# JessicaLeu-code/MotionPlanning_5D_m

Measured on AMD Instinct MI355X. Metric: CFS iterations/sec, 5-DoF 30-wp 8-obs batch-1024; l_inf wp err vs quadprog, higher is better.
Workload: dtype f64

## Files before the change

include/cfs_hip.h:

```cpp
#ifndef CFS_HIP_H
#define CFS_HIP_H

#ifdef __cplusplus
extern "C" {
#endif

#define CFS_ABI_VERSION 1
#define CFS_MAX_LINKS 8
#define CFS_MAX_OBS 32
#define CFS_MAX_H 64

typedef enum cfs_error {
    CFS_SUCCESS = 0,
    CFS_ERR_INVALID_ARG = -1,
    CFS_ERR_NO_DEVICE = -2,
    CFS_ERR_HIP = -3,
    CFS_ERR_NOT_SPD = -4,
    CFS_ERR_DYNAMICS = -5,
    CFS_ERR_ALLOC = -6
} cfs_error;

typedef enum cfs_status {
    CFS_OK_CONVERGED = 0,
    CFS_OK_MAXITER = 1,
// ... 295 lines not shown
int cfs_cart_path_mesh(const cfs_cart_desc *d, int nmesh, const cfs_mesh *const *meshes, const double *D_mesh, int flags, int T,
                       const double *start, const int *start_state, const double *target_pos, const double *target_axis,
                       const double *theta_ref, const cfs_cart_out *out);
int cfs_cart_path_mesh_device(const cfs_cart_desc *d, int nmesh, const cfs_mesh *const *meshes, const double *D_mesh ,
                              int flags, int T, const double *start, const int *start_state, const double *target_pos,
                              const double *target_axis, const double *theta_ref, const cfs_cart_out *out, void *stream);

int cfs_cart_follow(const cfs_cart_desc *d, int T, int npts, const double *start, const int *start_state, const double *path_pos,
                    const double *path_axis, const double *theta_ref, const cfs_cart_out *out);
int cfs_cart_follow_device(const cfs_cart_desc *d, int T, int npts, const double *start, const int *start_state, const double *path_pos,
                           const double *path_axis, const double *theta_ref, const cfs_cart_out *out, void *stream);
int cfs_cart_follow_mesh(const cfs_cart_desc *d, int nmesh, const cfs_mesh *const *meshes, const double *D_mesh, int flags, int T, int npts,
                         const double *start, const int *start_state, const double *path_pos, const double *path_axis,
                         const double *theta_ref, const cfs_cart_out *out);
int cfs_cart_follow_mesh_device(const cfs_cart_desc *d, int nmesh, const cfs_mesh *const *meshes, const double *D_mesh ,
                                int flags, int T, int npts, const double *start, const int *start_state, const double *path_pos,
                                const double *path_axis, const double *theta_ref, const cfs_cart_out *out, void *stream);

#define CFS_DBG_NO_REFINE 2
#define CFS_DBG_NO_WARM_START 8
#define CFS_DBG_NO_CERTIFICATE 16
#define CFS_DBG_NO_PRUNE 32
#define CFS_DBG_NO_AUTO_ORDER 64
#define CFS_DBG_TIER_W1 128
#define CFS_DBG_CLEAR_NO_BOUND 256
#define CFS_DBG_CLEAR_SEED 512
int cfs_debug_set_options(cfs_problem *p, int mask, int warm_max, double polish_tol);
int cfs_debug_fused_tier(int njoint, int H, int nobs, int mode, int per_waypoint, int limits, int force_w1, int *tier);
int cfs_debug_stamps(cfs_problem *p, int B, unsigned long long *out);
int cfs_debug_trace_begin(cfs_problem *p, int b, int cap);
int cfs_debug_trace_read(cfs_problem *p, double *out);
int cfs_debug_log_u(cfs_problem *p, int on);
int cfs_debug_read_u_log(cfs_problem *p, int B, double *out);
int cfs_debug_rrt_frontier_overflows(unsigned long long *count, int reset);
int cfs_debug_ik_frontier_overflows(unsigned long long *count, int reset);
int cfs_debug_cart_frontier_overflows(unsigned long long *count, int reset);

#ifdef __cplusplus
}
#endif
#endif
```

motionplanning_5d_m_amd/_lib.py:

```python
from __future__ import annotations

import ctypes as C
import os

try:
    import torch
except Exception:
    torch = None

_HERE = os.path.dirname(os.path.abspath(__file__))
LIB_PATH = os.path.join(_HERE, "libcfs_hip.so")

CFS_MAX_LINKS = 8
CFS_MAX_OBS = 32
CFS_MAX_H = 64

CFS_SUCCESS = 0
ERRORS = {-1: "CFS_ERR_INVALID_ARG", -2: "CFS_ERR_NO_DEVICE", -3: "CFS_ERR_HIP", -4: "CFS_ERR_NOT_SPD",
          -5: "CFS_ERR_DYNAMICS", -6: "CFS_ERR_ALLOC"}
STATUS = {0: "OK_CONVERGED", 1: "OK_MAXITER", 2: "QP_INFEASIBLE", 3: "NUMERIC", 4: "SOFT_ENDED"}
ROBOT_KIND = {"M16iB": 0, "M200i": 1, "2L": 2}
MODE = {"CFS": 0, "PSGCFS": 1}
JACOBIAN = {"fd_literal": 0, "analytic": 1}
INFEASIBLE = {"stop": 0, "soften": 1}
# ... 211 lines not shown
    ("cfs_solve_batch_device", C.c_int, [_P, C.POINTER(cfs_batch_in), C.POINTER(cfs_batch_out), _P]),
    ("cfs_set_state_cost", C.c_int, [_P, _P]),
    ("cfs_build_terms_device", C.c_int, [_P, C.c_int, _P, _P, _P, _P, _P, _P, _P]),
    ("cfs_build_terms_from_routes_device", C.c_int, [_P, C.c_int, _P, C.c_int, _P, _P, _P, _P, _P]),
    ("cfs_profile_enable", C.c_int, [_P, C.c_int]),
    ("cfs_profile_read", C.c_int, [_P, C.POINTER(C.c_double), C.POINTER(C.c_double), C.POINTER(C.c_int)]),
    ("cfs_dist_arm", C.c_int, [C.POINTER(cfs_robot), C.c_int, C.c_int, _P, C.c_int, _P, _P, _P, _P]),
    ("cfs_linearize", C.c_int, [_P, C.c_int, _P, _P, _P, _P, _P]),
    ("cfs_get_con", C.c_int, [_P, C.c_int, _P, _P, _P, _P, _P, _P]),
    ("cfs_qp", C.c_int, [_P, C.c_int, _P, _P, _P, _P, _P, _P, _P, _P, _P]),
    ("cfs_mesh_create", C.c_int, [_P, C.c_int, _P, C.c_int, C.POINTER(_P)]),
    ("cfs_mesh_load_stl", C.c_int, [C.c_char_p, C.c_double, C.c_int, C.POINTER(_P)]),
    ("cfs_mesh_info", C.c_int, [_P, C.POINTER(C.c_int), C.POINTER(C.c_int), C.POINTER(C.c_int), C.POINTER(C.c_double)]),
    ("cfs_mesh_destroy", None, [_P]),
    ("cfs_mesh_segment_distance", C.c_int, [_P, C.c_int, _P, _P, _P, _P]),
    ("cfs_dist_arm_mesh", C.c_int, [C.POINTER(cfs_robot), C.c_int, C.c_int, _P, _P, _P, _P, _P]),
    ("cfs_problem_set_meshes", C.c_int, [_P, C.c_int, _P]),
    ("cfs_problem_set_mesh_motion", C.c_int, [_P, _P]),
    ("cfs_chomp_batch", C.c_int, [_P, C.POINTER(cfs_batch_in), _P, _P, _P, C.POINTER(cfs_batch_out)]),
    ("cfs_build_terms_from_ragged_routes_device", C.c_int, [_P, C.c_int, _P, C.c_int, _P, _P, _P, _P, _P, _P]),
    ("cfs_rrt_grow", C.c_int, [C.POINTER(cfs_rrt_desc), C.c_int, C.POINTER(cfs_rrt_out)]),
    ("cfs_rrt_grow_device", C.c_int, [C.POINTER(cfs_rrt_desc), C.c_int, C.POINTER(cfs_rrt_out), _P]),
    ("cfs_rrt_grow_mesh", C.c_int, [C.POINTER(cfs_rrt_desc), C.c_int, _P, _P, C.c_int, C.c_int, C.POINTER(cfs_rrt_out)]),
    ("cfs_rrt_grow_mesh_device", C.c_int, [C.POINTER(cfs_rrt_desc), C.c_int, _P, _P, C.c_int, C.c_int, C.POINTER(cfs_rrt_out), _P]),
    ("cfs_cost_b", C.c_int, [_P, C.c_int, _P, _P, _P, _P]),
    ("cfs_get_cost", C.c_int, [_P, C.c_int, _P, _P, _P, _P]),
    ("cfs_debug_set_options", C.c_int, [_P, C.c_int, C.c_int, C.c_double]),
    ("cfs_debug_fused_tier", C.c_int, [C.c_int] * 7 + [C.POINTER(C.c_int)]),
    ("cfs_debug_stamps", C.c_int, [_P, C.c_int, _P]),
    ("cfs_debug_trace_begin", C.c_int, [_P, C.c_int, C.c_int]),
    ("cfs_debug_trace_read", C.c_int, [_P, _P]),
    ("cfs_debug_log_u", C.c_int, [_P, C.c_int]),
    ("cfs_debug_read_u_log", C.c_int, [_P, C.c_int, _P]),
    ("cfs_debug_rrt_frontier_overflows", C.c_int, [C.POINTER(C.c_ulonglong), C.c_int]),
    ("cfs_problem_set_jacobian", C.c_int, [_P, C.c_int]),
    ("cfs_problem_get_jacobian", C.c_int, [_P, C.POINTER(C.c_int)]),
    ("cfs_problem_set_infeasible_policy", C.c_int, [_P, C.c_int, C.c_double]),
    ("cfs_problem_get_infeasible_policy", C.c_int, [_P, C.POINTER(C.c_int), C.POINTER(C.c_double)]),
    ("cfs_soft_results", C.c_int, [_P, C.c_int, _P, _P]),
    ("cfs_dist_arm_grad", C.c_int, [C.POINTER(cfs_robot), C.c_int, C.c_int, _P, C.c_int, _P, _P, _P, _P]),
    ("cfs_select_best_device", C.c_int, [_P, C.c_int, C.c_int, _P, C.POINTER(cfs_batch_out), _P, C.POINTER(cfs_batch_out), _P, _P, _P, _P]),
    ("cfs_problem_set_obstacle_motion", C.c_int, [_P, C.c_int]),
    ("cfs_problem_get_obstacle_motion", C.c_int, [_P, C.POINTER(C.c_int)]),
    ("cfs_problem_set_joint_limits", C.c_int, [_P, _P, _P]),
    ("cfs_problem_get_joint_limits", C.c_int, [_P, C.POINTER(C.c_int), _P, _P]),
    ("cfs_clearance_device", C.c_int, [_P, C.c_int, C.c_int, _P, _P, _P, _P, _P, _P, _P, _P, _P, _P]),
    ("cfs_clearance", C.c_int, [_P, C.c_int, C.c_int, _P, _P, _P, _P, _P, _P, _P, _P, _P]),
    ("cfs_clearance_mesh_device", C.c_int, [_P, C.c_int, C.c_int, _P, _P, _P, _P, _P, _P, _P, _P, _P, _P, _P]),
    ("cfs_clearance_mesh", C.c_int, [_P, C.c_int, C.c_int, _P, _P, _P, _P, _P, _P, _P, _P, _P, _P]),
    ("cfs_clearance_mesh_motion_device", C.c_int, [_P, C.c_int, C.c_int, _P, _P, _P, _P, _P, _P, _P, _P, _P, _P, _P]),
    ("cfs_clearance_mesh_motion", C.c_int, [_P, C.c_int, C.c_int, _P, _P, _P, _P, _P, _P, _P, _P, _P, _P]),
    ("cfs_ik_solve", C.c_int, [C.POINTER(cfs_ik_desc), C.c_int, _P, _P, _P, C.POINTER(cfs_ik_out)]),
    ("cfs_ik_solve_device", C.c_int, [C.POINTER(cfs_ik_desc), C.c_int, _P, _P, _P, C.POINTER(cfs_ik_out), _P]),
    ("cfs_tool_pose", C.c_int, [C.POINTER(cfs_robot), C.c_int, _P, _P, C.c_int, _P, _P, _P, _P]),
    ("cfs_ik_solve_mesh", C.c_int, [C.POINTER(cfs_ik_desc), C.c_int, _P, _P, C.c_int, C.c_int, _P, _P, _P, C.POINTER(cfs_ik_out)]),
    ("cfs_ik_solve_mesh_device", C.c_int, [C.POINTER(cfs_ik_desc), C.c_int, _P, _P, C.c_int, C.c_int, _P, _P, _P, C.POINTER(cfs_ik_out), _P]),
    ("cfs_debug_ik_frontier_overflows", C.c_int, [C.POINTER(C.c_ulonglong), C.c_int]),
    ("cfs_cart_path", C.c_int, [C.POINTER(cfs_cart_desc), C.c_int, _P, _P, _P, _P, _P, C.POINTER(cfs_cart_out)]),
    ("cfs_cart_path_device", C.c_int, [C.POINTER(cfs_cart_desc), C.c_int, _P, _P, _P, _P, _P, C.POINTER(cfs_cart_out), _P]),
    ("cfs_cart_path_mesh", C.c_int, [C.POINTER(cfs_cart_desc), C.c_int, _P, _P, C.c_int, C.c_int, _P, _P, _P, _P, _P, C.POINTER(cfs_cart_out)]),
    ("cfs_cart_path_mesh_device", C.c_int, [C.POINTER(cfs_cart_desc), C.c_int, _P, _P, C.c_int, C.c_int, _P, _P, _P, _P, _P, C.POINTER(cfs_cart_out),
                                            _P]),
    ("cfs_debug_cart_frontier_overflows", C.c_int, [C.POINTER(C.c_ulonglong), C.c_int]),
    ("cfs_cart_follow", C.c_int, [C.POINTER(cfs_cart_desc), C.c_int, C.c_int, _P, _P, _P, _P, _P, C.POINTER(cfs_cart_out)]),
    ("cfs_cart_follow_device", C.c_int, [C.POINTER(cfs_cart_desc), C.c_int, C.c_int, _P, _P, _P, _P, _P, C.POINTER(cfs_cart_out), _P]),
    ("cfs_cart_follow_mesh", C.c_int, [C.POINTER(cfs_cart_desc), C.c_int, _P, _P, C.c_int, C.c_int, C.c_int, _P, _P, _P, _P, _P,
# ... 38 lines not shown
```

motionplanning_5d_m_amd/csrc/cfs_api.hip:

```cpp
#include "cfs_problem.h"
#include <cmath>
#include <cstdarg>
#include <cstdio>
#include <cstring>
#include <cstdlib>
#include <new>
#include <vector>

namespace {

thread_local char g_err[512] = "";
int g_device = 0;

int have_device()
{
    int n = 0;
    if (hipGetDeviceCount(&n) != hipSuccess) return 0;
    return n;
}

}

int cfs_fail(int code, const char *fmt, ...)
{
// ... 137 lines not shown
    if (FamilyRefusal r = check_double_integrator(nj, H, dt, desc->Aaug, desc->Baug)) return cfs_fail(r.code, "%s", r.text);
    if (have_device() == 0) return cfs_fail(CFS_ERR_NO_DEVICE, "no HIP device visible");
    FamilyMatrices fm;
    if (FamilyRefusal r = family_matrices(nj, H, dt, desc->mode, desc->QQ, fm)) return cfs_fail(r.code, "%s", r.text);
    cfs_problem *p = new (std::nothrow) cfs_problem();
    if (!p) return cfs_fail(CFS_ERR_ALLOC, "out of host memory");
    p->d = *desc;
    p->QQ_host.assign(desc->QQ, desc->QQ + (size_t)nn * nn);
    p->d.QQ = p->d.Aaug = p->d.Baug = p->d.lim = p->d.MAX_input = p->d.margin = nullptr;
    p->device = g_device;
    if (hipDeviceGetAttribute(&p->n_cu, hipDeviceAttributeMultiprocessorCount, g_device) != hipSuccess || p->n_cu < 1) p->n_cu = 256;
    p->nn = nn; p->ns = ns; p->nx = nx; p->lmax_vel = fm.lmax_vel; p->lmax_H = fm.lmax_H;
    cfs_build_dev_robot(desc->robot, p->hrobot);
    cfs_clear_build_rho(p->hrobot, nj, p->rho);
    const size_t Bm = (size_t)desc->max_batch;
    p->pool_n = (int)std::min<size_t>(Bm, (size_t)2 * p->n_cu);
    const size_t Pn = (size_t)p->pool_n;
    hipError_t e = hipSetDevice(p->device);
    auto up = [&](auto &buf, const auto *src, size_t count) { if (e == hipSuccess) e = buf.upload(src, count); };
    auto room = [&](auto &buf, size_t count) { if (e == hipSuccess) e = buf.alloc(count); };
    up(p->rb, &p->hrobot, 1); up(p->QQ, desc->QQ, (size_t)nn * nn); up(p->Hinv, fm.Hinv.data(), (size_t)nn * nn);
    up(p->M1n, fm.M1n.data(), (size_t)nn * nn); up(p->M2n, fm.M2n.data(), (size_t)nn * nn); up(p->Hq, fm.Hq.data(), (size_t)nn * nn);
    room(p->Pt, Pn * pt_stride(nn));
    room(p->lim, 3 * (size_t)nj);
    if (e == hipSuccess) e = hipMemcpy(p->lim.p, desc->lim, nj * sizeof(double), hipMemcpyHostToDevice);
    if (desc->mode == CFS_MODE_CFS) up(p->maxin, desc->MAX_input, nn);
    else if (e == hipSuccess) e = p->maxin.zeros(nn);
    up(p->margin, desc->margin, desc->nobs);
    room(p->x0, Bm * nn); room(p->qu, Bm * nn); room(p->dist, Bm * desc->nobs * H); room(p->grad, Bm * desc->nobs * H * nj);
    room(p->Yg, Pn * nn * nn);
    if (e == hipSuccess) e = p->pool_flag.zeros(Pn * 16);
    if (desc->mode == CFS_MODE_CFS) { room(p->u_hist, Bm * (size_t)desc->MAX_O_ITER * nn); room(p->qu_hist, Bm * (size_t)desc->MAX_O_ITER * nn); }
    room(p->noise_row, Bm); room(p->linkid, Bm * desc->nobs * H); room(p->order, Bm); room(p->okey, Bm); room(p->order_user, Bm);
    if (e != hipSuccess) {
        delete p;
        return cfs_fail(CFS_ERR_HIP, "device setup failed: %s", hipGetErrorString(e));
    }
    *out = p;
    return CFS_SUCCESS;
}

void cfs_problem_destroy(cfs_problem *p)
{
    if (!p) return;
    (void)hipSetDevice(p->device);
    delete p;
}

int cfs_problem_family(const cfs_problem *p, double *QQ, double *alpha)
{
    if (!p) return cfs_fail(CFS_ERR_INVALID_ARG, "NULL handle");
    if (QQ) memcpy(QQ, p->QQ_host.data(), p->QQ_host.size() * sizeof(double));
    if (alpha) *alpha = p->d.alpha;
    return CFS_SUCCESS;
}

int cfs_problem_create_from_weights(const cfs_problem_desc *desc, const cfs_cost_weights *w, cfs_problem **out)
{
    if (!desc || !w || !out) return cfs_fail(CFS_ERR_INVALID_ARG, "NULL argument");
    *out = nullptr;
    if (!w->Qp || !w->Qv || !w->Rblk) return cfs_fail(CFS_ERR_INVALID_ARG, "Qp/Qv/Rblk must be given");
    const int nj = desc->njoint, H = desc->H;
    if (nj < 2 || nj > 6 || H < 1 || H > CFS_MAX_H) return cfs_fail(CFS_ERR_INVALID_ARG, "njoint %d / H %d unsupported", nj, H);
    const double dt = desc->robot.delta_t;
    if (!(dt > 0)) return cfs_fail(CFS_ERR_INVALID_ARG, "robot.delta_t must be positive");
    WeightFamily wf;
// ... 87 lines not shown
int cfs_solve_batch_device(cfs_problem *p, const cfs_batch_in *in, const cfs_batch_out *out, void *stream)
{
    if (!p || !in || !out) return cfs_fail(CFS_ERR_INVALID_ARG, "NULL argument");
    const int B = in->B;
    if (int rc = cfs_check_batch(p, B)) return rc;
    if (!in->x_init || !in->xR1 || !in->ff || !in->caug || !in->obs) return cfs_fail(CFS_ERR_INVALID_ARG, "NULL input array");
    if (!out->u || !out->x_ || !out->cost_all || !out->e_cost_all || !out->e_u_all || !out->iter_O || !out->total_iter || !out->status)
        return cfs_fail(CFS_ERR_INVALID_ARG, "NULL output array");
    CFS_HIPCHK(hipSetDevice(p->device));
    hipStream_t s = reinterpret_cast<hipStream_t>(stream);

    hipEvent_t e4[4] = {nullptr, nullptr, nullptr, nullptr};
    int rc = CFS_SUCCESS;
    if (p->prof)
        for (int k = 0; k < 4 && rc == CFS_SUCCESS; ++k) {
            if (!p->ev_free.empty()) { e4[k] = p->ev_free.back(); p->ev_free.pop_back(); }
            else if (hipEventCreate(&e4[k]) != hipSuccess) { e4[k] = nullptr; rc = cfs_fail(CFS_ERR_HIP, "hipEventCreate failed"); }
        }
    if (rc == CFS_SUCCESS) {
        rc = enqueue_solve(p, in, out, s, e4);
        if (rc != CFS_SUCCESS) p->pool_dirty = true;
    }
    if (p->prof)
        for (int k = 0; k < 4; ++k)
            if (e4[k]) (rc == CFS_SUCCESS ? p->ev : p->ev_free).push_back(e4[k]);
    return rc;
}

static int enqueue_solve(cfs_problem *p, const cfs_batch_in *in, const cfs_batch_out *out, hipStream_t s, hipEvent_t *e4)
{
    const int B = in->B, nj = p->d.njoint, nn = p->nn, K = p->d.MAX_O_ITER;
    if (p->pool_dirty) {
        CFS_HIPCHK(hipMemsetAsync(p->pool_flag.p, 0, (size_t)p->pool_n * 16 * sizeof(int), s));
        p->pool_dirty = false;
    }
    if (p->prof) CFS_HIPCHK(hipEventRecord(e4[0], s));
    if (p->d.mode == CFS_MODE_CFS) {
        GemvParams g;
        g.B = B; g.nn = nn; g.M = p->Hinv.p; g.X = in->ff; g.Y = p->x0.p; g.scale = -1.0;
        launch_batched_gemv(g, s);
    }
    if (p->prof) CFS_HIPCHK(hipEventRecord(e4[1], s));
    FusedParams fp;
    fill_fused_family(p, fp, B);
    fp.noise_rows = in->noise ? in->noise_rows : 0;
    fp.x_init = in->x_init; fp.xR1 = in->xR1; fp.ff = in->ff; fp.caug = in->caug; fp.obs = in->obs; fp.noise = in->noise;
    fp.u = out->u; fp.x_ = out->x_; fp.cost_all = out->cost_all; fp.e_cost_all = out->e_cost_all; fp.e_u_all = out->e_u_all;
    fp.iter_O = out->iter_O; fp.total_iter = out->total_iter; fp.status = out->status;
    fp.u_hist = (p->d.mode == CFS_MODE_CFS && K > 0) ? p->u_hist.p : nullptr;
    const int nline = p->d.nobs - p->nmesh;
    if (p->order_mode == 1 && p->order_n == B) fp.order = p->order_user.p;
    else if (p->order_mode != 2 && !(p->dbg_mask & CFS_DBG_NO_AUTO_ORDER) && B > p->n_cu && nline > 0) {
        OrderParams op;
        op.rb = p->rb.p; op.B = B; op.H = p->d.H; op.nj = nj; op.nobs = nline; op.obs_stride = p->d.nobs;
        op.wp_stride = cfs_moving(p) ? p->d.nobs : 0;
        op.x_init = in->x_init; op.obs = in->obs; op.margin = p->margin.p; op.key = p->okey.p; op.order = p->order.p;
        launch_order(op, s);
        fp.order = p->order.p;
    }
    SoftParams sp;
    const SoftParams *soft = soft_params(p, sp, true);
    if (p->soft_viol.p) {
        CFS_HIPCHK(hipMemsetAsync(p->soft_viol.p, 0, (size_t)B * std::max(K, 1) * sizeof(double), s));
        CFS_HIPCHK(hipMemsetAsync(p->soft_n.p, 0, (size_t)B * sizeof(int), s));
    }
    if (p->prof) CFS_HIPCHK(hipEventRecord(e4[2], s));
    if (p->nmesh == 0) {
        CFS_HIPCHK(launch_fused(nj, fp, s, force_w1(p), analytic(p), soft, cfs_moving(p), limited(p)));
    } else {
        LinMeshParams lm = lin_mesh_params(p, B);
        fp.nmesh = p->nmesh; fp.ext_dist = p->dist.p; fp.ext_grad = p->grad.p; fp.max_launch_iters = 1;
        fp.st_qu = p->qu.p; fp.st_cost = p->mesh.st_cost.p; fp.st_noise = p->noise_row.p; fp.st_done = p->mesh.st_done.p;
        for (int it = 0; it < std::max(K, 1); ++it) {
            lm.x_ = it == 0 ? in->x_init : out->x_;
            lm.status_done = it == 0 ? nullptr : p->mesh.st_done.p;
            lm.seed_prev = it > 0;
            CFS_HIPCHK(launch_linearize_mesh(nj, lm, s));
            fp.resume = it > 0;
            CFS_HIPCHK(launch_fused(nj, fp, s, force_w1(p), analytic(p), nullptr, false, limited(p)));
        }
    }
    if (p->prof) CFS_HIPCHK(hipEventRecord(e4[3], s));
    if (fp.u_hist) {
        if (p->u_hist.n) {
            GemvParams g;
            g.B = B * K; g.nn = nn; g.M = p->QQ.p; g.X = p->u_hist.p; g.Y = p->qu_hist.p; g.scale = 1.0;
            launch_batched_gemv(g, s);
            CostHistParams ch;
            ch.B = B; ch.nn = nn; ch.max_o_iter = K; ch.u_hist = p->u_hist.p; ch.qu_hist = p->qu_hist.p;
            ch.ff = in->ff; ch.caug = in->caug; ch.iter_O = out->iter_O; ch.cost_all = out->cost_all; ch.e_cost_all = out->e_cost_all;
// ... 154 lines not shown
    return CFS_SUCCESS;
}

int cfs_debug_trace_read(cfs_problem *p, double *out)
{
    if (!p || !out) return cfs_fail(CFS_ERR_INVALID_ARG, "NULL argument");
    if (!p->trace.p) return cfs_fail(CFS_ERR_INVALID_ARG, "no trace was begun");
    CFS_HIPCHK(hipSetDevice(p->device));
    CFS_HIPCHK(hipDeviceSynchronize());
    CFS_HIPCHK(hipMemcpy(out, p->trace.p, (size_t)(p->trace_cap + 1) * 8 * sizeof(double), hipMemcpyDeviceToHost));
    return CFS_SUCCESS;
}

int cfs_debug_log_u(cfs_problem *p, int on)
{
    if (!p) return cfs_fail(CFS_ERR_INVALID_ARG, "NULL handle");
    CFS_HIPCHK(hipSetDevice(p->device));
    CFS_HIPCHK(hipDeviceSynchronize());
    p->u_log.release();
    if (!on || p->d.MAX_O_ITER < 1) return CFS_SUCCESS;
    const size_t n = (size_t)p->d.max_batch * p->d.MAX_O_ITER * p->nn;
    CFS_HIPCHK(p->u_log.zeros(n));
    return CFS_SUCCESS;
}

int cfs_debug_read_u_log(cfs_problem *p, int B, double *out)
{
    if (!p || !out) return cfs_fail(CFS_ERR_INVALID_ARG, "NULL argument");
    if (!p->u_log.p) return cfs_fail(CFS_ERR_INVALID_ARG, "the u log is not enabled");
    if (int rc = cfs_check_batch(p, B)) return rc;
    CFS_HIPCHK(hipSetDevice(p->device));
    CFS_HIPCHK(hipDeviceSynchronize());
    CFS_HIPCHK(hipMemcpy(out, p->u_log.p, (size_t)B * p->d.MAX_O_ITER * p->nn * sizeof(double), hipMemcpyDeviceToHost));
    return CFS_SUCCESS;
}

int cfs_set_state_cost(cfs_problem *p, const double *Qaug)
{
    if (!p || !Qaug) return cfs_fail(CFS_ERR_INVALID_ARG, "NULL argument");
    CFS_HIPCHK(hipSetDevice(p->device));
    std::vector<double> F1, F2, Cq;
    state_cost_terms(p->d.njoint, p->d.H, p->d.robot.delta_t, Qaug, F1, F2, Cq);
    CFS_HIPCHK(p->F1.upload(F1.data(), F1.size())); CFS_HIPCHK(p->F2.upload(F2.data(), F2.size())); CFS_HIPCHK(p->Cq.upload(Cq.data(), Cq.size()));
    return CFS_SUCCESS;
}

static int build_terms(cfs_problem *p, int B, const double *x0, const double *xg, const double *route, int nwp, const int *nwp_b, int nwp_stride,
                       double *x_init, double *xR1, double *ff, double *caug, void *stream)
{
    if (!p->F1.p) return cfs_fail(CFS_ERR_INVALID_ARG, "call cfs_set_state_cost first");
    CFS_HIPCHK(hipSetDevice(p->device));
    TermsParams t;
    t.B = B; t.H = p->d.H; t.nj = p->d.njoint; t.F1 = p->F1.p; t.F2 = p->F2.p; t.Cq = p->Cq.p;
    t.x0 = x0; t.xg = xg; t.route = route; t.nwp = nwp; t.nwp_b = nwp_b; t.nwp_stride = nwp_stride; t.dt = p->d.robot.delta_t;
    t.x_init = x_init; t.xR1 = xR1; t.ff = ff; t.caug = caug;
    launch_build_terms(t, reinterpret_cast<hipStream_t>(stream));
    CFS_HIPCHK(hipGetLastError());
    return CFS_SUCCESS;
}

int cfs_build_terms_device(cfs_problem *p, int B, const double *x0, const double *xg,
                           double *x_init, double *xR1, double *ff, double *caug, void *stream)
{
    if (!p || !x0 || !xg || !x_init || !xR1 || !ff || !caug) return cfs_fail(CFS_ERR_INVALID_ARG, "NULL argument");
    if (B < 1) return cfs_fail(CFS_ERR_INVALID_ARG, "B must be >= 1");
    return build_terms(p, B, x0, xg, nullptr, 0, nullptr, 0, x_init, xR1, ff, caug, stream);
// ... 406 lines not shown
```

motionplanning_5d_m_amd/csrc/cfs_device.h:

```cpp
#pragma once
#include <hip/hip_runtime.h>
#include <stdint.h>
#include "../../include/cfs_hip.h"

#define CFS_WAVE 64

struct DevRobot {
    int kind;
    int nlink;
    double dh_d[CFS_MAX_LINKS];
    double dh_a[CFS_MAX_LINKS];
    double ca[CFS_MAX_LINKS];
    double sa[CFS_MAX_LINKS];
    double th_off[CFS_MAX_LINKS];
    double base[3];
    double cap[CFS_MAX_LINKS * 6];
    double t2l[CFS_MAX_LINKS * 3];
    double shift_bound;
    double prune_tol;
};
static_assert(sizeof(DevRobot) % 8 == 0, "DevRobot is copied to LDS as doubles");

struct DevCost {
    double Qp[36], Qv[36], Rs[36];
    double qc, ws, wt, pad;
};
static_assert(sizeof(DevCost) % 8 == 0, "DevCost is read as doubles");

struct DistArmParams {
    const DevRobot *rb;
    int N, nobs, nj;
    const double *theta;
    const double *obs;
    double *d;
    int *linkid;
    double *pos;
    double *grad;
};
void launch_dist_arm(const DistArmParams &p, hipStream_t s);
void launch_dist_arm_grad(const DistArmParams &p, hipStream_t s);

struct OrderParams {
    const DevRobot *rb;
    int B, H, nj, nobs;
    int obs_stride;
    int wp_stride;
    const double *x_init;
    const double *obs;
    const double *margin;
    int *key;
    int *order;
};
void launch_order(const OrderParams &p, hipStream_t s);

struct DenseConParams {
    int B, H, nj, nobs;
    double dt;
    const double *dist, *grad;
    const double *u;
    const double *xR1;
    const double *lim, *margin;
    double *Ainq;
    double *binq;
    const double *plim;
};
void launch_dense_con(const DenseConParams &p, hipStream_t s);

struct ClearParams {
    const DevRobot *rb;
    int B, H, nj, nobs, S;
    int move;
    double dt;
    const double *x_, *u, *xR1, *obs;
    double *dist_wp, *dist_path, *dist_lower, *t_path;
    int *link_path;
    int obs_stride, out_stride;
    double rho[CFS_MAX_LINKS * CFS_MAX_LINKS];
};
hipError_t launch_clearance(const ClearParams &p, hipStream_t s);
void cfs_clear_build_rho(const DevRobot &rb, int nj, double *rho);

enum { QP_OK = 0, QP_INFEASIBLE = 2, QP_NUMERIC = 3 };

struct GemvParams {
    int B, nn;
    const double *M;
// ... 89 lines not shown
```

motionplanning_5d_m_amd/csrc/cfs_geom.hip:

```cpp
#include "cfs_geom_dev.h"
#include "cfs_host.h"

namespace {

__global__ __launch_bounds__(256) void cfs_dist_arm_kernel(DistArmParams P)
{
    __shared__ __attribute__((aligned(16))) double s_rb[sizeof(DevRobot) / 8];
    {
        const double *src = reinterpret_cast<const double *>(P.rb);
        for (int e = threadIdx.x; e < (int)(sizeof(DevRobot) / 8); e += blockDim.x) s_rb[e] = src[e];
    }
    __syncthreads();
    const DevRobot *rb = reinterpret_cast<const DevRobot *>(s_rb);
    const int n = blockIdx.x * blockDim.x + threadIdx.x;
    if (n >= P.N) return;
    double ends[CFS_MAX_LINKS * 6];
    double M[12], Mn[12];
    for (int k = 0; k < P.nj; ++k) {
        double sn, cs;
        sincos(P.theta[(size_t)n * P.nj + k] - rb->th_off[k], &sn, &cs);
        fk_step(rb, k, sn, cs, k == 0 ? nullptr : M, Mn);
        for (int q = 0; q < 12; ++q) M[q] = Mn[q];
        link_ends(rb, k, M, ends + k * 6);
        if (P.pos) for (int q = 0; q < 6; ++q) P.pos[((size_t)n * P.nj + k) * 6 + q] = ends[k * 6 + q];
    }
    for (int j = 0; j < P.nobs; ++j) {
        double o6[6];
        for (int q = 0; q < 6; ++q) o6[q] = P.obs[j * 6 + q];
        double d = INFINITY;
        int lid = 0;
        for (int k = 0; k < P.nj; ++k) {
            const double dis = seg_seg_dist(ends + k * 6, o6);
            if (dis < d) { d = dis; lid = k + 1; }
        }
// ... 5 lines not shown
__global__ __launch_bounds__(256) void cfs_dist_arm_grad_kernel(DistArmParams P)
{
    __shared__ __attribute__((aligned(16))) double s_rb[sizeof(DevRobot) / 8];
    {
        const double *src = reinterpret_cast<const double *>(P.rb);
        for (int e = threadIdx.x; e < (int)(sizeof(DevRobot) / 8); e += blockDim.x) s_rb[e] = src[e];
    }
    __syncthreads();
    const DevRobot *rb = reinterpret_cast<const DevRobot *>(s_rb);
    const int n = blockIdx.x * blockDim.x + threadIdx.x;
    if (n >= P.N) return;
    double sc[CFS_MAX_LINKS * 2], ends[CFS_MAX_LINKS * 6], tw[CFS_MAX_LINKS * 6];
    for (int k = 0; k < P.nj; ++k) sincos(P.theta[(size_t)n * P.nj + k] - rb->th_off[k], &sc[2 * k], &sc[2 * k + 1]);
    arm_chain(rb, P.nj, sc, ends, tw);
    for (int j = 0; j < P.nobs; ++j) {
        double o6[6];
        for (int q = 0; q < 6; ++q) o6[q] = P.obs[j * 6 + q];
        double d = INFINITY;
        int lid = 0;
        for (int k = 0; k < P.nj; ++k) {
            const double dis = seg_seg_dist(ends + k * 6, o6);
            if (dis < d) { d = dis; lid = k + 1; }
        }
        const size_t o = (size_t)n * P.nobs + j;
        P.d[o] = d;
        P.linkid[o] = lid;
        double *g = P.grad + o * P.nj;
        if (lid > 0) winner_grad(ends + (lid - 1) * 6, tw, lid - 1, P.nj, o6, g);
        else for (int m = 0; m < P.nj; ++m) g[m] = 0.0;
    }
}

constexpr int ORDER_PB = 8;
__global__ __launch_bounds__(256, 4) void cfs_order_key_kernel(OrderParams P)
{
    __shared__ __attribute__((aligned(16))) double s_rb[sizeof(DevRobot) / 8];
    __shared__ int s_cnt[ORDER_PB];
    {
        const double *src = reinterpret_cast<const double *>(P.rb);
        for (int e = threadIdx.x; e < (int)(sizeof(DevRobot) / 8); e += blockDim.x) s_rb[e] = src[e];
    }
    if (threadIdx.x < ORDER_PB) s_cnt[threadIdx.x] = 0;
    __syncthreads();
    const DevRobot *rb = reinterpret_cast<const DevRobot *>(s_rb);
    const int sub = threadIdx.x >> 5, lane = threadIdx.x & 31;
    const int b = blockIdx.x * ORDER_PB + sub, ns = 2 * P.nj;
    int cnt = 0;
    if (b < P.B)
    for (int i = lane; i < P.H; i += 32) {
        double ends[CFS_MAX_LINKS * 6];
        double M[12], Mn[12];
        for (int k = 0; k < P.nj; ++k) {
            double sn, cs;
            sincos(P.x_init[((size_t)b * P.H + i) * ns + k] - rb->th_off[k], &sn, &cs);
            fk_step(rb, k, sn, cs, k == 0 ? nullptr : M, Mn);
            for (int q = 0; q < 12; ++q) M[q] = Mn[q];
            link_ends(rb, k, M, ends + k * 6);
        }
        const double *ob = P.obs + ((size_t)b * P.obs_stride * (P.wp_stride ? P.H : 1) + (size_t)i * P.wp_stride) * 6;
        for (int j = 0; j < P.nobs; ++j) {
            double o6[6];
            for (int q = 0; q < 6; ++q) o6[q] = ob[j * 6 + q];
            double d = INFINITY;
            for (int k = 0; k < P.nj; ++k) d = fmin(d, seg_seg_dist(ends + k * 6, o6));
            cnt += d < P.margin[j];
        }
    }
    if (cnt) atomicAdd(&s_cnt[sub], cnt);
    __syncthreads();
    if (lane == 0 && b < P.B) P.key[b] = s_cnt[sub];
}

__global__ __launch_bounds__(256) void cfs_order_rank_kernel(OrderParams P)
{
    const int i = blockIdx.x * blockDim.x + threadIdx.x;
    const int ki = i < P.B ? P.key[i] : 0;
    int rank = 0;
    for (int j = 0; j < P.B; ++j) {
        const int kj = P.key[j];
        rank += (kj > ki) || (kj == ki && j < i);
    }
    if (i < P.B) P.order[rank] = i;
}

__global__ __launch_bounds__(256) void cfs_dense_con_kernel(DenseConParams P)
{
    const int nj = P.nj, H = P.H, nn = H * nj, ns = 2 * nj;
    const int per = 1 + 2 * nj, rref = P.nobs * H * per, rows = rref + (P.plim ? 2 * nn : 0);
    const int b = blockIdx.y, col = blockIdx.x;
    const int k = col / nj, cc = col % nj;
    const double dt = P.dt;
    double *A = P.Ainq + ((size_t)b * rows * nn) + (size_t)col * rows;
    const double *g = P.grad + (size_t)b * P.nobs * H * nj;
    for (int r = threadIdx.x; r < rref; r += blockDim.x) {
        const int blk = r / per, t = r % per, j = blk / H, i = blk % H;
        double v = 0.0;
        if (k <= i) {
            if (t == 0) v = -(g[((size_t)j * H + i) * nj + cc] * ((double)(i - k) + 0.5) * dt * dt);
            else if (t <= nj) v = (t - 1 == cc) ? dt : 0.0;
            else v = (t - 1 - nj == cc) ? -dt : 0.0;
        }
        if (v == 0.0) v = 0.0;
        A[r] = v;
    }
    for (int r = rref + threadIdx.x; r < rows; r += blockDim.x) {
        const int q = r - rref, kk = q % nn, i = kk / nj, c = kk % nj;
        double v = (c == cc && k <= i) ? ((double)(i - k) + 0.5) * dt * dt : 0.0;
        if (q >= nn) v = -v;
        if (v == 0.0) v = 0.0;
        A[r] = v;
    }
    if (col == 0) {
        const double *u = P.u + (size_t)b * nn;
// ... 8 lines not shown
            double s;
            if (t == 0) {
                double gbu = 0.0;
                for (int c = 0; c < nj; ++c) {
                    double pu = 0.0;
                    for (int kk = 0; kk <= i; ++kk) pu += ((double)(i - kk) + 0.5) * dt * dt * u[kk * nj + c];
                    gbu += g[((size_t)j * H + i) * nj + c] * pu;
                }
                s = (P.dist[((size_t)b * P.nobs + j) * H + i] - P.margin[j]) - gbu;
            } else {
                const int c = (t - 1) % nj;
                const double v0 = x1[nj + c];
                s = (t <= nj) ? P.lim[c] - v0 : P.lim[c] + v0;
            }
            P.binq[(size_t)b * rows + r] = s;
        }
    }
}

}

void launch_dist_arm(const DistArmParams &p, hipStream_t s)
{
    const dim3 grid((p.N + 255) / 256), block(256);
    hipLaunchKernelGGL(cfs_dist_arm_kernel, grid, block, 0, s, p);
}

void launch_dist_arm_grad(const DistArmParams &p, hipStream_t s)
{
    const dim3 grid((p.N + 255) / 256), block(256);
    hipLaunchKernelGGL(cfs_dist_arm_grad_kernel, grid, block, 0, s, p);
}

void launch_order(const OrderParams &p, hipStream_t s)
{
    hipLaunchKernelGGL(cfs_order_key_kernel, dim3((p.B + ORDER_PB - 1) / ORDER_PB), dim3(256), 0, s, p);
    hipLaunchKernelGGL(cfs_order_rank_kernel, dim3((p.B + 255) / 256), dim3(256), 0, s, p);
}

void launch_dense_con(const DenseConParams &p, hipStream_t s)
{
    const dim3 grid(p.H * p.nj, p.B), block(256);
    hipLaunchKernelGGL(cfs_dense_con_kernel, grid, block, 0, s, p);
}

static int dist_arm(const cfs_robot *robot, int njoint, int N, const double *theta, int nobs, const double *obs, double *d, int *linkid, double *pos,
                    double *grad, bool with_grad)
{
    int rc = cfs_check_robot(robot, njoint);
    if (rc) return rc;
    if (N < 0 || nobs < 0 || !theta || !obs || !d || (with_grad && (!linkid || !grad))) return cfs_fail(CFS_ERR_INVALID_ARG, "bad argument");
    if (N == 0 || nobs == 0) return CFS_SUCCESS;
    rc = cfs_use_device(cfs_current_device());
    if (rc) return rc;
    DevRobot hr;
    cfs_build_dev_robot(*robot, hr);
    const size_t n = (size_t)N * nobs;
    Stage st;
    DistArmParams P;
    P.rb = st.up(&hr, 1);
    P.N = N; P.nobs = nobs; P.nj = njoint;
    P.theta = st.up(theta, (size_t)N * njoint);
    P.obs = st.up(obs, (size_t)nobs * 6);
    P.d = st.out<double>(n);
    P.linkid = st.out<int>(n);
    P.pos = pos ? st.out<double>((size_t)N * njoint * 6) : nullptr;
    P.grad = with_grad ? st.out<double>(n * njoint) : nullptr;
    if (st.err != hipSuccess) return st.result("staging");
    if (with_grad) launch_dist_arm_grad(P, nullptr);
    else launch_dist_arm(P, nullptr);
// ... 18 lines not shown
```

motionplanning_5d_m_amd/csrc/cfs_problem.h:

```cpp
#pragma once
#include "cfs_host.h"

struct MeshSet {
    DevBuf<DevMesh> meshes_d;
    std::vector<DevMesh> meshes_h;
    std::vector<double> mesh_frame;
    DevBuf<double> st_cost, m_ends, m_base, m_shift, m_upper, m_pd, m_pnd;
    DevBuf<int> st_done, m_tri, m_near, m_pi;
};
struct MeshMotion {
    DevBuf<double> mesh_pose;
    DevBuf<double> mesh_itv;
    DevBuf<double> cmm_pose, cmm_v;
    int cmm_S = 0, cmm_cap = 0, cmm_gen = -1;
    int turn_mesh = -1, turn_wp = 0;
};
struct ClearMeshWork {
    DevBuf<double> cm_d, cm_L, cm_rho;
    DevBuf<int> cm_lk, cm_tri, cm_seed;
    int S = 0;
};

struct cfs_problem {
    cfs_problem_desc d;
    int device;
    int nn, ns, nx;
    double lmax_vel, lmax_H;
    DevRobot hrobot;
    DevBuf<DevRobot> rb;
    DevBuf<double> QQ, Hinv, Hq, M1n, M2n, lim, maxin, margin;
    DevBuf<double> F1, F2, Cq;
    DevBuf<DevCost> cost;
    std::vector<double> QQ_host;
    DevBuf<double> x0, qu, dist, grad, Yg, Pt, u_hist, qu_hist;
    DevBuf<int> noise_row, linkid, pool_flag;
    bool pool_dirty = false;
    int pool_n = 1;
    DevBuf<int> order, okey;
    DevBuf<int> order_user;
    int n_cu = 256;
    int order_mode = 0, order_n = 0;
    int nmesh = 0;
    MeshSet mesh;
    MeshMotion mm;
    int motion_gen = 0;
    ClearMeshWork cm;
    int dbg_mask = 0, dbg_warm_max = 0;
    double dbg_polish_tol = 1e-11;
    DevBuf<unsigned long long> stamps;
    int stamps_B = 0;
    DevBuf<double> trace;
    int trace_b = -1, trace_cap = 0;
    DevBuf<double> u_log;
    int jac = CFS_JAC_FD_LITERAL;
    int infeas = CFS_INFEAS_STOP;
    int motion = CFS_OBS_STATIC;
    bool limited = false;
    std::vector<double> jlim;
    double rho[CFS_MAX_LINKS * CFS_MAX_LINKS];
    double soft_weight = 0.0;
    DevBuf<double> soft_viol;
    DevBuf<int> soft_n;
    bool prof = false;
    std::vector<hipEvent_t> ev;
    std::vector<hipEvent_t> ev_free;
    void reset_mesh_motion() { mm = MeshMotion{}; ++motion_gen; }
    ~cfs_problem()
    {
        for (hipEvent_t e : ev) (void)hipEventDestroy(e);
        for (hipEvent_t e : ev_free) (void)hipEventDestroy(e);
    }
};
// ... 19 lines not shown
```

motionplanning_5d_m_amd/solvers.py:

```python
from __future__ import annotations

import ctypes as C
import math
from types import SimpleNamespace

import numpy as np

from . import _args, _lib
from ._args import f64 as _f64, obs_meshes, ptr as _ptr
from .robotproperty2 import to_c_robot

try:
    import torch
except Exception:
    torch = None


def obs_to_array(obs):
    return _f64(np.stack([np.zeros(6) if "mesh" in o else
                          np.concatenate([np.asarray(o["l"], float)[:, 0], np.asarray(o["l"], float)[:, 1]]) for o in obs]))


def obs_moving(obs):
    return any("mesh" not in o and np.ndim(o["l"]) == 3 for o in obs)
# ... 482 lines not shown
    def debug_options(self, warm_max=0, polish_tol=0.0, **flags):
        mask = 0
        for k, v in flags.items():
            if v:
                mask |= _lib.DBG[k]
        _lib.check(self._lib.cfs_debug_set_options(self._h, mask, int(warm_max), float(polish_tol)))

    def stamps(self, B=None):
        if B is not None:
            _lib.check(self._lib.cfs_debug_stamps(self._h, int(B), None))
            self._stamps_B = int(B)
            return None
        out = np.zeros((self._stamps_B, 12), np.uint64)
        _lib.check(self._lib.cfs_debug_stamps(self._h, self._stamps_B, _ptr(out)))
        return out

    def trace(self, b=None, cap=0):
        if b is not None:
            _lib.check(self._lib.cfs_debug_trace_begin(self._h, int(b), int(cap)))
            self._trace_cap = int(cap)
            return None
        buf = np.zeros((self._trace_cap + 1) * 8)
        _lib.check(self._lib.cfs_debug_trace_read(self._h, _ptr(buf)))
        return buf[8:8 + 8 * int(buf[0])].reshape(-1, 8)

    def log_u(self, on=True):
        _lib.check(self._lib.cfs_debug_log_u(self._h, 1 if on else 0))

    def read_u_log(self, B):
        out = np.zeros((B, self.K, self.nn))
        _lib.check(self._lib.cfs_debug_read_u_log(self._h, int(B), _ptr(out)))
        return out

    def linearize(self, x_, obs):
        x_, obs = _f64(x_), _f64(obs)
        B = x_.shape[0]
        self._check_obs(obs, B)
        dist = np.zeros((B, self.nobs, self.H))
        lid = np.zeros((B, self.nobs, self.H), np.int32)
        grad = np.zeros((B, self.nobs, self.H, self.nj))
        _lib.check(self._lib.cfs_linearize(self._h, B, _ptr(x_), _ptr(obs), _ptr(dist), _ptr(lid), _ptr(grad)))
        return dist, lid, grad

    def get_con(self, x_, u, xR1, obs):
        x_, u, xR1, obs = _f64(x_), _f64(u), _f64(xR1), _f64(obs)
        B = x_.shape[0]
        self._check_obs(obs, B)
        A = np.zeros((B, self.nn, self.rows))
        b = np.zeros((B, self.rows))
        _lib.check(self._lib.cfs_get_con(self._h, B, _ptr(x_), _ptr(u), _ptr(xR1), _ptr(obs), _ptr(A), _ptr(b)))
        return A.transpose(0, 2, 1), b

    def qp(self, lin, u_lin, xR1, dist, grad, want_lambda=True):
        lin, u_lin, xR1, dist, grad = _f64(lin), _f64(u_lin), _f64(xR1), _f64(dist), _f64(grad)
        B = lin.shape[0]
        u = np.zeros((B, self.nn))
        nlam = self.nobs * self.H + (4 if self.joint_limits() is None else 6) * self.nn
        lam = np.zeros((B, nlam)) if want_lambda else None
        it, st = np.zeros(B, np.int32), np.zeros(B, np.int32)
        _lib.check(self._lib.cfs_qp(self._h, B, _ptr(lin), _ptr(u_lin), _ptr(xR1), _ptr(dist), _ptr(grad), _ptr(u),
                                    _ptr(lam), _ptr(it), _ptr(st)))
        return u, lam, it, st


FUSED_TIERS = ("w1", "w2m", "w2s")

# ... 203 lines not shown
```

Before: 11.34 million.

## Fold launch-order sort into key kernel via last-block counting sort

The launch-order pre-pass used to run a key kernel and then an O(B^2) rank kernel that read keys from global memory. The key kernel now has a templated fold path: the last block to arrive, detected with an atomic ticket, builds a stable counting sort over key bins in shared memory and writes the order directly, so the second launch is gone. The fallback rank kernel now tiles keys through shared memory as int4. This adds an atomic arrival counter, fences, and a serial tail on one block, plus debug APIs for inspecting the chosen path.

```diff
diff --git a/include/cfs_hip.h b/include/cfs_hip.h
--- a/include/cfs_hip.h
+++ b/include/cfs_hip.h
@@ -351,6 +351,9 @@
 int cfs_debug_trace_read(cfs_problem *p, double *out);
 int cfs_debug_log_u(cfs_problem *p, int on);
 int cfs_debug_read_u_log(cfs_problem *p, int B, double *out);
+int cfs_debug_launch_order(cfs_problem *p, int B, int *key, int *order);
+int cfs_debug_launch_order_bins(cfs_problem *p, int cap);
+int cfs_debug_launch_order_path(const cfs_problem *p, int B, int *path, int *last);
 int cfs_debug_rrt_frontier_overflows(unsigned long long *count, int reset);
 int cfs_debug_ik_frontier_overflows(unsigned long long *count, int reset);
 int cfs_debug_cart_frontier_overflows(unsigned long long *count, int reset);
diff --git a/motionplanning_5d_m_amd/_lib.py b/motionplanning_5d_m_amd/_lib.py
--- a/motionplanning_5d_m_amd/_lib.py
+++ b/motionplanning_5d_m_amd/_lib.py
@@ -267,6 +267,9 @@
     ("cfs_debug_trace_read", C.c_int, [_P, _P]),
     ("cfs_debug_log_u", C.c_int, [_P, C.c_int]),
     ("cfs_debug_read_u_log", C.c_int, [_P, C.c_int, _P]),
+    ("cfs_debug_launch_order", C.c_int, [_P, C.c_int, _P, _P]),
+    ("cfs_debug_launch_order_bins", C.c_int, [_P, C.c_int]),
+    ("cfs_debug_launch_order_path", C.c_int, [_P, C.c_int, C.POINTER(C.c_int), C.POINTER(C.c_int)]),
     ("cfs_debug_rrt_frontier_overflows", C.c_int, [C.POINTER(C.c_ulonglong), C.c_int]),
     ("cfs_problem_set_jacobian", C.c_int, [_P, C.c_int]),
     ("cfs_problem_get_jacobian", C.c_int, [_P, C.POINTER(C.c_int)]),
diff --git a/motionplanning_5d_m_amd/csrc/cfs_api.hip b/motionplanning_5d_m_amd/csrc/cfs_api.hip
--- a/motionplanning_5d_m_amd/csrc/cfs_api.hip
+++ b/motionplanning_5d_m_amd/csrc/cfs_api.hip
@@ -193,6 +193,7 @@
     if (e == hipSuccess) e = p->pool_flag.zeros(Pn * 16);
     if (desc->mode == CFS_MODE_CFS) { room(p->u_hist, Bm * (size_t)desc->MAX_O_ITER * nn); room(p->qu_hist, Bm * (size_t)desc->MAX_O_ITER * nn); }
     room(p->noise_row, Bm); room(p->linkid, Bm * desc->nobs * H); room(p->order, Bm); room(p->okey, Bm); room(p->order_user, Bm);
+    if (e == hipSuccess) e = p->order_arrive.zeros(1);
     if (e != hipSuccess) {
         delete p;
         return cfs_fail(CFS_ERR_HIP, "device setup failed: %s", hipGetErrorString(e));
@@ -346,8 +347,10 @@
     const int B = in->B, nj = p->d.njoint, nn = p->nn, K = p->d.MAX_O_ITER;
     if (p->pool_dirty) {
         CFS_HIPCHK(hipMemsetAsync(p->pool_flag.p, 0, (size_t)p->pool_n * 16 * sizeof(int), s));
+        CFS_HIPCHK(hipMemsetAsync(p->order_arrive.p, 0, sizeof(int), s));
         p->pool_dirty = false;
     }
+    p->order_last = 0;
     if (p->prof) CFS_HIPCHK(hipEventRecord(e4[0], s));
     if (p->d.mode == CFS_MODE_CFS) {
         GemvParams g;
@@ -369,7 +372,9 @@
         op.rb = p->rb.p; op.B = B; op.H = p->d.H; op.nj = nj; op.nobs = nline; op.obs_stride = p->d.nobs;
         op.wp_stride = cfs_moving(p) ? p->d.nobs : 0;
         op.x_init = in->x_init; op.obs = in->obs; op.margin = p->margin.p; op.key = p->okey.p; op.order = p->order.p;
-        launch_order(op, s);
+        op.arrive = p->order_arrive.p; op.cap = p->order_cap;
+        p->order_last = launch_order(op, s);
+        p->order_last_B = B;
         fp.order = p->order.p;
     }
     SoftParams sp;
@@ -590,6 +595,35 @@
     CFS_HIPCHK(hipSetDevice(p->device));
     CFS_HIPCHK(hipDeviceSynchronize());
     CFS_HIPCHK(hipMemcpy(out, p->u_log.p, (size_t)B * p->d.MAX_O_ITER * p->nn * sizeof(double), hipMemcpyDeviceToHost));
+    return CFS_SUCCESS;
+}
+
+int cfs_debug_launch_order(cfs_problem *p, int B, int *key, int *order)
+{
+    if (!p || !key || !order) return cfs_fail(CFS_ERR_INVALID_ARG, "NULL argument");
+    if (int rc = cfs_check_batch(p, B)) return rc;
+    if (!p->order_last) return cfs_fail(CFS_ERR_INVALID_ARG, "the last solve of this handle did not run the automatic launch-order pre-pass");
+    if (B != p->order_last_B) return cfs_fail(CFS_ERR_INVALID_ARG, "B=%d, but the last solve ordered %d problems", B, p->order_last_B);
+    CFS_HIPCHK(hipSetDevice(p->device));
+    CFS_HIPCHK(hipDeviceSynchronize());
+    CFS_HIPCHK(hipMemcpy(key, p->okey.p, (size_t)B * sizeof(int), hipMemcpyDeviceToHost));
+    CFS_HIPCHK(hipMemcpy(order, p->order.p, (size_t)B * sizeof(int), hipMemcpyDeviceToHost));
+    return CFS_SUCCESS;
+}
+
+int cfs_debug_launch_order_bins(cfs_problem *p, int cap)
+{
+    if (!p) return cfs_fail(CFS_ERR_INVALID_ARG, "NULL handle");
+    p->order_cap = cap > 0 ? cap : CFS_ORDER_BINS;
+    return CFS_SUCCESS;
+}
+
+int cfs_debug_launch_order_path(const cfs_problem *p, int B, int *path, int *last)
+{
+    if (!p || !path) return cfs_fail(CFS_ERR_INVALID_ARG, "NULL argument");
+    if (B < 1) return cfs_fail(CFS_ERR_INVALID_ARG, "B must be >= 1");
+    *path = cfs_order_path(B, p->d.H, p->d.nobs - p->nmesh, p->order_cap);
+    if (last) *last = p->order_last;
     return CFS_SUCCESS;
 }
 
diff --git a/motionplanning_5d_m_amd/csrc/cfs_device.h b/motionplanning_5d_m_amd/csrc/cfs_device.h
--- a/motionplanning_5d_m_amd/csrc/cfs_device.h
+++ b/motionplanning_5d_m_amd/csrc/cfs_device.h
@@ -50,8 +50,12 @@
     const double *margin;
     int *key;
     int *order;
+    int *arrive;
+    int cap;
 };
-void launch_order(const OrderParams &p, hipStream_t s);
+constexpr int CFS_ORDER_BINS = 4096;
+int launch_order(const OrderParams &p, hipStream_t s);
+int cfs_order_path(int B, int H, int nline, int cap);
 
 struct DenseConParams {
     int B, H, nj, nobs;
diff --git a/motionplanning_5d_m_amd/csrc/cfs_geom.hip b/motionplanning_5d_m_amd/csrc/cfs_geom.hip
--- a/motionplanning_5d_m_amd/csrc/cfs_geom.hip
+++ b/motionplanning_5d_m_amd/csrc/cfs_geom.hip
@@ -1,5 +1,7 @@
 #include "cfs_geom_dev.h"
 #include "cfs_host.h"
+#include <algorithm>
+#include <climits>
 
 namespace {
 
@@ -71,10 +73,16 @@
 }
 
 constexpr int ORDER_PB = 8;
+#ifndef CFS_ORDER_FOLD
+#define CFS_ORDER_FOLD 1
+#endif
+template <bool FOLD>
 __global__ __launch_bounds__(256, 4) void cfs_order_key_kernel(OrderParams P)
 {
     __shared__ __attribute__((aligned(16))) double s_rb[sizeof(DevRobot) / 8];
     __shared__ int s_cnt[ORDER_PB];
+    __shared__ int s_hist[FOLD ? CFS_ORDER_BINS : 1];
+    __shared__ int s_wsum[4], s_last;
     {
         const double *src = reinterpret_cast<const double *>(P.rb);
         for (int e = threadIdx.x; e < (int)(sizeof(DevRobot) / 8); e += blockDim.x) s_rb[e] = src[e];
@@ -108,16 +116,104 @@
     if (cnt) atomicAdd(&s_cnt[sub], cnt);
     __syncthreads();
     if (lane == 0 && b < P.B) P.key[b] = s_cnt[sub];
-}
-
+    if constexpr (FOLD) {
+        asm volatile("s_waitcnt vmcnt(0)" ::: "memory");
+        __syncthreads();
+        if (threadIdx.x == 0) {
+            __builtin_amdgcn_fence(__ATOMIC_RELEASE, "agent");
+            const int ticket = __hip_atomic_fetch_add(P.arrive, 1, __ATOMIC_RELAXED, __HIP_MEMORY_SCOPE_AGENT);
+            const int last = ticket == (int)gridDim.x - 1;
+            if (last) {
+                __builtin_amdgcn_fence(__ATOMIC_ACQUIRE, "agent");
+                asm volatile("s_waitcnt vmcnt(0)" ::: "memory");
+                __hip_atomic_store(P.arrive, 0, __ATOMIC_RELAXED, __HIP_MEMORY_SCOPE_AGENT);
+            }
+            s_last = last;
+        }
+        __syncthreads();
+        if (!s_last) return;
+        const int B = P.B, nbins = P.H * P.nobs + 1;
+        const int W = min(4, CFS_ORDER_BINS / nbins), n = W * nbins;
+        const int nchunk = (B + 63) >> 6, cpw = (nchunk + W - 1) / W;
+        for (int e = threadIdx.x; e < n; e += 256) s_hist[e] = 0;
+        __syncthreads();
+        for (int j = threadIdx.x; j < B; j += 256) {
+            const int k = min(max(P.key[j], 0), nbins - 1);
+            atomicAdd(&s_hist[(nbins - 1 - k) * W + (j >> 6) / cpw], 1);
+        }
+        __syncthreads();
+        {
+            const int per = (n + 255) >> 8, lo = threadIdx.x * per, hi = min(lo + per, n), wv = threadIdx.x >> 6, ln = threadIdx.x & 63;
+            int sum = 0;
+            for (int e = lo; e < hi; ++e) sum += s_hist[e];
+            int incl = sum;
+            for (int d = 1; d < 64; d <<= 1) {
+                const int up = __shfl_up(incl, d, 64);
+                if (ln >= d) incl += up;
+            }
+            if (ln == 63) s_wsum[wv] = incl;
+            __syncthreads();
+            int excl = incl - sum;
+            for (int w = 0; w < wv; ++w) excl += s_wsum[w];
+            for (int e = lo; e < hi; ++e) {
+                const int c = s_hist[e];
+                s_hist[e] = excl;
+                excl += c;
+            }
+        }
+        __syncthreads();
+        const int wv = threadIdx.x >> 6, ln = threadIdx.x & 63;
+        if (wv >= W) return;
+        for (int c = wv * cpw; c < min((wv + 1) * cpw, nchunk); ++c) {
+            const int j = c * 64 + ln;
+            bool todo = j < B;
+            const int k = todo ? min(max(P.key[j], 0), nbins - 1) : 0;
+            unsigned long long live;
+            while ((live = __ballot(todo)) != 0) {
+                const int lead = __ffsll((long long)live) - 1;
+                const int kk = __shfl(k, lead, 64);
+                const bool mine = todo && k == kk;
+                const unsigned long long eq = __ballot(mine);
+                int *cur = &s_hist[(nbins - 1 - kk) * W + wv];
+                const int base = *cur;
+                if (mine) P.order[base + __popcll(eq & ((1ull << ln) - 1))] = j;
+                if (ln == lead) *cur = base + __popcll(eq);
+                todo = todo && !mine;
+            }
+        }
+    }
+}
+
+constexpr int ORDER_TILE = 4096;
 __global__ __launch_bounds__(256) void cfs_order_rank_kernel(OrderParams P)
 {
+    __shared__ int4 s_key[ORDER_TILE / 4];
     const int i = blockIdx.x * blockDim.x + threadIdx.x;
     const int ki = i < P.B ? P.key[i] : 0;
     int rank = 0;
-    for (int j = 0; j < P.B; ++j) {
-        const int kj = P.key[j];
-        rank += (kj > ki) || (kj == ki && j < i);
+    for (int t0 = 0; t0 < P.B; t0 += ORDER_TILE) {
+        const int nt = min(ORDER_TILE, P.B - t0);
+        for (int q = threadIdx.x; q < ORDER_TILE / 4; q += 256) {
+            int4 v;
+            if (4 * q + 4 <= nt) v = *reinterpret_cast<const int4 *>(P.key + t0 + 4 * q);
+            else {
+                int e[4];
+                for (int r = 0; r < 4; ++r) e[r] = 4 * q + r < nt ? P.key[t0 + 4 * q + r] : INT_MIN;
+                v = make_int4(e[0], e[1], e[2], e[3]);
+            }
+            s_key[q] = v;
+        }
+        __syncthreads();
+        const int nq = (nt + 3) >> 2;
+        for (int q = 0; q < nq; ++q) {
+            const int4 v = s_key[q];
+            const int j = t0 + 4 * q;
+            rank += (v.x > ki) || (v.x == ki && j < i);
+            rank += (v.y > ki) || (v.y == ki && j + 1 < i);
+            rank += (v.z > ki) || (v.z == ki && j + 2 < i);
+            rank += (v.w > ki) || (v.w == ki && j + 3 < i);
+        }
+        __syncthreads();
     }
     if (i < P.B) P.order[rank] = i;
 }
@@ -192,10 +288,22 @@
     hipLaunchKernelGGL(cfs_dist_arm_grad_kernel, grid, block, 0, s, p);
 }
 
-void launch_order(const OrderParams &p, hipStream_t s)
-{
-    hipLaunchKernelGGL(cfs_order_key_kernel, dim3((p.B + ORDER_PB - 1) / ORDER_PB), dim3(256), 0, s, p);
-    hipLaunchKernelGGL(cfs_order_rank_kernel, dim3((p.B + 255) / 256), dim3(256), 0, s, p);
+int cfs_order_path(int B, int H, int nline, int cap)
+{
+    (void)B;
+    return (CFS_ORDER_FOLD && H * nline + 1 <= std::min(cap, CFS_ORDER_BINS)) ? 1 : 2;
+}
+
+int launch_order(const OrderParams &p, hipStream_t s)
+{
+    const int path = cfs_order_path(p.B, p.H, p.nobs, p.cap);
+    const dim3 grid((p.B + ORDER_PB - 1) / ORDER_PB), block(256);
+    if (path == 1) hipLaunchKernelGGL(cfs_order_key_kernel<true>, grid, block, 0, s, p);
+    else {
+        hipLaunchKernelGGL(cfs_order_key_kernel<false>, grid, block, 0, s, p);
+        hipLaunchKernelGGL(cfs_order_rank_kernel, dim3((p.B + 255) / 256), block, 0, s, p);
+    }
+    return path;
 }
 
 void launch_dense_con(const DenseConParams &p, hipStream_t s)
diff --git a/motionplanning_5d_m_amd/csrc/cfs_problem.h b/motionplanning_5d_m_amd/csrc/cfs_problem.h
--- a/motionplanning_5d_m_amd/csrc/cfs_problem.h
+++ b/motionplanning_5d_m_amd/csrc/cfs_problem.h
@@ -38,6 +38,9 @@
     int pool_n = 1;
     DevBuf<int> order, okey;
     DevBuf<int> order_user;
+    DevBuf<int> order_arrive;
+    int order_cap = CFS_ORDER_BINS;
+    int order_last = 0, order_last_B = 0;
     int n_cu = 256;
     int order_mode = 0, order_n = 0;
     int nmesh = 0;
diff --git a/motionplanning_5d_m_amd/solvers.py b/motionplanning_5d_m_amd/solvers.py
--- a/motionplanning_5d_m_amd/solvers.py
+++ b/motionplanning_5d_m_amd/solvers.py
@@ -538,6 +538,19 @@
         _lib.check(self._lib.cfs_debug_read_u_log(self._h, int(B), _ptr(out)))
         return out
 
+    def launch_order(self, B):
+        key, order = np.zeros(B, np.int32), np.zeros(B, np.int32)
+        _lib.check(self._lib.cfs_debug_launch_order(self._h, int(B), _ptr(key), _ptr(order)))
+        return key, order
+
+    def launch_order_bins(self, cap=0):
+        _lib.check(self._lib.cfs_debug_launch_order_bins(self._h, int(cap)))
+
+    def launch_order_path(self, B):
+        path, last = C.c_int(0), C.c_int(0)
+        _lib.check(self._lib.cfs_debug_launch_order_path(self._h, int(B), C.byref(path), C.byref(last)))
+        return path.value, last.value
+
     def linearize(self, x_, obs):
         x_, obs = _f64(x_), _f64(obs)
         B = x_.shape[0]
```

Measured after the change: 11.40 million (median of 6 runs). About the same (+0.5%).
